# telegraphroad/VCNF

Hardware: AMD Instinct MI355X
Metric: flow transforms/sec (log_prob + sample), D=64 RQ-spline, batch=1M (higher is better)
Workload: dtype f32 results on fp16x3 split operands: every fp32 operand of a conditioner GEMM travels as hi + lo fp16 halves, three f16 matrix instructions per product (four in the 48- and 16-deep layers), fp32 accumulation; measured against fp64 (tests/test_gpu_gemm_error.py): GEMM error 0.6-0.75x the exact-fp32

## Files before the change

### vcnf_amd/csrc/fused_layer_v6.hip

```cpp
#include <hip/hip_runtime.h>
#include <stdint.h>

#include "../../include/vcnf_hip.h"
#include "rqs_math.hpp"
#include "fused_common.hpp"
#include "rqs_lean.hpp"
#include "split_half.hpp"

#ifndef VCNF_ABL
#define VCNF_ABL 0
#endif
#ifndef VCNF_TIME
#define VCNF_TIME 0
#endif
#ifndef VCNF_AHEAD
#define VCNF_AHEAD 1
#endif
#if VCNF_TIME
#define VCNF_T(I) { const long long t_ = clock64(); tacc[I] += t_ - tlast; tlast = t_; }
#define VCNF_TIME_PARAM , float* tstamps
#define VCNF_TIME_ARG , time_buffer()
#else
#define VCNF_T(I)
#define VCNF_TIME_PARAM
#define VCNF_TIME_ARG
#endif

#define VCNF_SYNC() { __builtin_amdgcn_sched_barrier(0); asm volatile("s_waitcnt lgkmcnt(0)\n\ts_barrier" ::: "memory"); __builtin_amdgcn_sched_barrier(0); }

namespace vcnf {

#if VCNF_TIME
constexpr int kTimeSlots = 24;
static float* time_buffer() {
  static float* buf = nullptr;
  if (!buf && hipMalloc(&buf, 2 * kTimeSlots * sizeof(float)) != hipSuccess) buf = nullptr;
  return buf;
}
extern "C" int vcnf_v6_phase_stamps(float* out) {
  if (!time_buffer() || hipDeviceSynchronize() != hipSuccess) return VCNF_ERR_LAUNCH;
  return hipMemcpy(out, time_buffer(), 2 * kTimeSlots * sizeof(float), hipMemcpyDeviceToHost) == hipSuccess ? VCNF_OK : VCNF_ERR_LAUNCH;
}
#endif

template <int DI, int DT, int C, int H, int NBLK, int K, bool INV>
__global__ __launch_bounds__(512, 2) void fused_rqs_layer_v6_kernel(const FusedArgs a VCNF_TIME_PARAM) {
  static_assert(H == 128 && K == 8, "4 row blocks of 32 over 4 waves; 3 K - 1 = 23 logits: two features per 48 rows");
  static_assert((DI == 16 || DI == 32) && DT == DI && (C == 0 || C == 16), "shape family");
  constexpr int kBlock = 512;
  constexpr int kTile = 128;
  constexpr int NCB = 4;
  constexpr int D = DI + DT;
  constexpr int XS = D + 4;
  constexpr int NTX = DI / 16;
  constexpr int NTC = C / 16;
  constexpr int NT0 = NTX + NTC;
  constexpr int NTH = H / 16;
  constexpr int P = 3 * K - 1;
  constexpr int NG = DT / 4;
  constexpr int NR = NG / 2;
  constexpr int TABW = 3 * (K + 1);
  using L = PackLayout6<DI, DT, C, H, NBLK, K>;
  constexpr int GFRAG = 3 * NTH * 2 * 64;
  constexpr int RING = VCNF_AHEAD + 1;

  extern __shared__ __align__(16) float smem[];
  uint4* act = reinterpret_cast<uint4*>(smem);
  uint4* act_hi = act;
  uint4* act_lo = act + NTH * NCB * 64;
  float* xt = smem + 2 * GFRAG * 4;
  uint4* ctxf = reinterpret_cast<uint4*>(xt + kTile * XS);
  float* tab = reinterpret_cast<float*>(ctxf + (C > 0 ? NCB * 2 * 64 : 0));
  float* ldt = tab + ((DI * TABW + 3) & ~3);
  int* tfi = reinterpret_cast<int*>(ldt + kTile);
  int* idi = tfi + DT;
  constexpr int NBV = C > 0 ? 3 : 2;
  constexpr int NBT = 1 + NBLK * NBV;
  constexpr int BPL = NG * 48 + NBT * (H / 2);
  float* biasf = reinterpret_cast<float*>(idi + DI + 4);
  int* tflag = reinterpret_cast<int*>(biasf + 2 * BPL);

  const int tid = threadIdx.x;
  const int lane = tid & 63;
  const int wave = __builtin_amdgcn_readfirstlane(tid >> 6);
  const int rp = wave & 3;
  const int ch = wave >> 2;
  const int c32 = lane & 31;
  const int kg = lane >> 5;
  const RqsConst& c = a.c;
  const bool shared = a.sh_w != nullptr;
  const LeanConst lc = make_lean_const(c);

  if (ch == 1) __builtin_amdgcn_s_setprio(1);
  for (int i = tid; i < NG * 96; i += kBlock) {
    const int g = i / 96, hf = i % 96 / 48;
    biasf[hf * BPL + g * 48 + i % 48] = a.wpack[L::BF + i];
  }
  for (int i = tid; i < NBT * H; i += kBlock) {
    const int v = i / H, blk = (v - 1) / NBV, sel = (v - 1) % NBV, r = i % H;
    const int off = v == 0 ? L::B0 : L::BLK0 + blk * L::BLK + (sel == 0 ? L::BA : sel == 1 ? L::BB : L::BC);
    biasf[(r >> 4 & 1) * BPL + NG * 48 + v * (H / 2) + (r >> 5) * 16 + (r & 15)] = a.wpack[off + r];
  }
  for (int i = tid; i < DT; i += kBlock) tfi[i] = a.tf_idx[i];
  for (int i = tid; i < DI; i += kBlock) idi[i] = a.id_idx[i];
  if (shared) {
    for (int i = tid; i < 3 * DI; i += kBlock) {
      const int f = i % DI;
      SplitLogits p{a.sh_w + f * K, a.sh_h + f * K, a.sh_d + f * (K - 1), K, 1.f, c.edge_logit, c.tails};
      rqs_build_table_part_k<K>(p, c, tab + f * TABW, 1, i / DI);
    }
  }

  const __amdgpu_buffer_rsrc_t wr =
      __builtin_amdgcn_make_buffer_rsrc(const_cast<float*>(a.wpack), 0, a.wpack_bytes, 0x00020000);
  const int voff = lane * 16;
  const float* bplane = biasf + kg * BPL;

  const long long ntiles = (a.B + kTile - 1) / kTile;
  bool bad = false;
  float satm = 0.f;
#if VCNF_TIME
  long long tacc[20], tlast = clock64();
  const long long tstart = tlast, rstart = wall_clock64();
  for (int i = 0; i < 20; ++i) tacc[i] = 0;
#endif
  float4 xpre[kTile * (D / 4) / kBlock], cpre[1];
  static_assert(kTile * (D / 4) % kBlock == 0 && (C == 0 || kTile * (C / 4) == kBlock), "rows per thread");
#define VCNF_PREFETCH_ROWS(TILE)                                                          \
  {                                                                                       \
    const long long pb0 = min((TILE) * kTile, a.B);                                       \
    const long long left = (a.B - pb0) * (D * 4);                                         \
    const __amdgpu_buffer_rsrc_t xr_ = __builtin_amdgcn_make_buffer_rsrc(                 \
        const_cast<float*>(a.x) + pb0 * D, 0, (int)min(left, (long long)(kTile * D * 4)), 0x00020000); \
    _Pragma("unroll") for (int k = 0; k < kTile * (D / 4) / kBlock; ++k)                  \
      xpre[k] = __builtin_bit_cast(float4, __builtin_amdgcn_raw_buffer_load_b128(xr_, (tid + kBlock * k) * 16, 0, 0)); \
    if (C > 0) {                                                                          \
      const long long leftc = (a.B - pb0) * (C * 4);                                      \
      const __amdgpu_buffer_rsrc_t cr_ = __builtin_amdgcn_make_buffer_rsrc(               \
          const_cast<float*>(a.ctx) + pb0 * C, 0, (int)min(leftc, (long long)(kTile * C * 4)), 0x00020000); \
      cpre[0] = __builtin_bit_cast(float4, __builtin_amdgcn_raw_buffer_load_b128(cr_, tid * 16, 0, 0)); \
    }                                                                                     \
  }
  VCNF_PREFETCH_ROWS((long long)blockIdx.x)
  for (long long tile = blockIdx.x; tile < ntiles; tile += gridDim.x) {
    const long long b0 = tile * kTile;
    const int rows = (int)min((long long)kTile, a.B - b0);
    satm = 0.f;
    { VCNF_T(0) VCNF_SYNC(); VCNF_T(15) }
    {
      constexpr int D4 = D / 4;
      if (tid == 0) *tflag = 0;
#pragma unroll
      for (int k = 0; k < kTile * D4 / kBlock; ++k) {
        const int i = tid + kBlock * k;
        const int r = i / D4, o = i - r * D4;
        *reinterpret_cast<float4*>(xt + r * XS + 4 * o) = xpre[k];
      }
      if (C > 0) {
        const int r = tid >> 2, part = tid & 3;
        half4 h4, l4;
        const float cv[4] = {cpre[0].x, cpre[0].y, cpre[0].z, cpre[0].w};
#pragma unroll
        for (int i = 0; i < 4; ++i) satm = fmaxf(satm, cv[i] == cv[i] ? __builtin_fabsf(cv[i]) : __builtin_inff());
        asm volatile("" : "+v"(satm));
#pragma unroll
        for (int i = 0; i < 4; ++i) {
          const float x = __builtin_amdgcn_fmed3f(cv[i], -65504.f, 65504.f);
          const _Float16 hv = (_Float16)x;
          h4[i] = hv;
          l4[i] = (_Float16)((x - (float)hv) * kLoScale);
        }
        const int at = (((r >> 5) * 2) * 64 + (r & 31) + 32 * (part >> 1));
        uint2* dh = reinterpret_cast<uint2*>(ctxf + at) + (part & 1);
        uint2* dl = reinterpret_cast<uint2*>(ctxf + at + 64) + (part & 1);
        *dh = __builtin_bit_cast(uint2, h4);
        *dl = __builtin_bit_cast(uint2, l4);
      }
    }
    { VCNF_T(1) VCNF_SYNC(); VCNF_T(15) }

    {
      constexpr int UNR = DI / 4;
      const int mi = tid >> 2, part = tid & 3;
      float lsum = 0.f;
      float xv[UNR], fv[UNR];
      float* px[UNR];
#pragma unroll
      for (int k = 0; k < UNR; ++k) {
        px[k] = xt + mi * XS + idi[part * UNR + k];
        xv[k] = *px[k];
        fv[k] = xv[k];
      }
      if (shared) {
        float yv[UNR], lad[UNR];
        bool in_[UNR];
#pragma unroll
        for (int k = 0; k < UNR; ++k) {
          in_[k] = (xv[k] >= c.lo_x) && (xv[k] <= c.hi_x);
          bool bad1 = false;
          rqs_point_table_inside<INV, K>(in_[k] ? xv[k] : c.lo_x, tab + (part * UNR + k) * TABW, yv[k], lad[k], bad1);
          bad = bad || (bad1 && in_[k]);
        }
#pragma unroll
        for (int k = 0; k < UNR; ++k) {
          const float o = in_[k] ? yv[k] : xv[k];
          *px[k] = o;
          if (INV) fv[k] = o;
          lsum += in_[k] ? lad[k] : 0.f;
        }
      }
      lsum += __shfl_xor(lsum, 1, 64);
      lsum += __shfl_xor(lsum, 2, 64);
      int tid_ = tid;
      asm volatile("" : "+v"(tid_));
      if (part == 0) ldt[tid_ >> 2] = lsum;
#pragma unroll
      for (int k = 0; k < UNR; ++k) satm = fmaxf(satm, fv[k] == fv[k] ? 0.f : __builtin_inff());
      const int k0 = part * UNR;
      const int t0 = k0 >> 4, kg0 = (k0 >> 3) & 1;
      const int at = (t0 * NCB + (mi >> 5)) * 64 + (mi & 31) + 32 * kg0;
      if (UNR == 8) {
        half8 h8, l8;
        float f8[8];
#pragma unroll
        for (int k = 0; k < 8; ++k) f8[k] = fv[k < UNR ? k : 0];
        split8<false>(f8, h8, l8, satm);
        act_hi[at] = __builtin_bit_cast(uint4, h8);
        act_lo[at] = __builtin_bit_cast(uint4, l8);
      } else {
        half4 h4, l4;
        satm = fmaxf(fmaxf(satm, __builtin_fabsf(fv[0])), __builtin_fabsf(fv[1]));
        satm = fmaxf(fmaxf(satm, __builtin_fabsf(fv[2 < UNR ? 2 : 0])), __builtin_fabsf(fv[3 < UNR ? 3 : 0]));
        asm volatile("" : "+v"(satm));
#pragma unroll
        for (int i = 0; i < 4; ++i) {
          const float x = __builtin_amdgcn_fmed3f(fv[i < UNR ? i : 0], -65504.f, 65504.f);
          const _Float16 hv = (_Float16)x;
          h4[i] = hv;
          l4[i] = (_Float16)((x - (float)hv) * kLoScale);
        }
        reinterpret_cast<uint2*>(act_hi + at)[(k0 >> 2) & 1] = __builtin_bit_cast(uint2, h4);
        reinterpret_cast<uint2*>(act_lo + at)[(k0 >> 2) & 1] = __builtin_bit_cast(uint2, l4);
      }
    }
    { VCNF_T(2) VCNF_SYNC(); VCNF_T(15) }
    if (ch == 1) { VCNF_T(14) VCNF_SYNC(); VCNF_T(16) }

    half8 ahi[NTH], alo[NTH];
    floatx16 abias;
#define VCNF_LOAD_BIAS16(DST, VEC)                                                        \
  _Pragma("unroll") for (int i_ = 0; i_ < 4; ++i_) {                                      \
    const floatx4 b4_ = *reinterpret_cast<const floatx4*>(bplane + NG * 48 + (VEC) * (H / 2) + 16 * rp + 4 * i_); \
    DST[4 * i_ + 0] = b4_[0]; DST[4 * i_ + 1] = b4_[1]; DST[4 * i_ + 2] = b4_[2]; DST[4 * i_ + 3] = b4_[3]; \
  }
#define VCNF_LOAD_HIDDEN(WOFF, BVEC)                                                      \
  {                                                                                       \
    _Pragma("unroll") for (int t = 0; t < NTH; ++t) {                                     \
      ahi[t] = __builtin_bit_cast(half8, wload(wr, voff, 4 * ((WOFF) + ((rp * NTH + t) * 2 + 0) * 256))); \
      alo[t] = __builtin_bit_cast(half8, wload(wr, voff, 4 * ((WOFF) + ((rp * NTH + t) * 2 + 1) * 256))); \
    }                                                                                     \
    VCNF_LOAD_BIAS16(abias, BVEC)                                                         \
  }

    floatx16 h[2];
    {
      half8 w0h[NT0], w0l[NT0];
      floatx16 bias0;
#pragma unroll
      for (int t = 0; t < NT0; ++t) {
        w0h[t] = __builtin_bit_cast(half8, wload(wr, voff, 4 * (L::W0 + ((rp * NT0 + t) * 2 + 0) * 256)));
        w0l[t] = __builtin_bit_cast(half8, wload(wr, voff, 4 * (L::W0 + ((rp * NT0 + t) * 2 + 1) * 256)));
      }
      VCNF_LOAD_BIAS16(bias0, 0)
#pragma unroll
      for (int j = 0; j < 2; ++j) {
        const int cb = 2 * ch + j;
        floatx16 mainv = bias0, corr = {}, corr2 = {};
#pragma unroll
        for (int t = 0; t < NT0; ++t) {
          const half8 bh = __builtin_bit_cast(half8, t < NTX ? act_hi[(t * NCB + cb) * 64 + lane] : ctxf[(cb * 2 + 0) * 64 + lane]);
          const half8 bl = __builtin_bit_cast(half8, t < NTX ? act_lo[(t * NCB + cb) * 64 + lane] : ctxf[(cb * 2 + 1) * 64 + lane]);
          mainv = mfma32h(w0h[t], bh, mainv);
          corr = mfma32h(w0h[t], bl, corr);
          corr = mfma32h(w0l[t], bh, corr);
          corr2 = mfma32h(w0l[t], bl, corr2);
        }
#pragma unroll
        for (int r = 0; r < 16; ++r) h[j][r] = fmaf(fmaf(corr2[r], kLoUnscale, corr[r]), kLoUnscale, mainv[r]);
      }
    }
    { VCNF_T(3) VCNF_SYNC(); VCNF_T(15) }
#define VCNF_PUBLISH(SRC, RELU)                                                           \
  _Pragma("unroll") for (int j = 0; j < 2; ++j) {                                         \
    _Pragma("unroll") for (int hh = 0; hh < 2; ++hh) {                                    \
      float v8_[8];                                                                       \
      _Pragma("unroll") for (int i = 0; i < 8; ++i) v8_[i] = SRC[j][8 * hh + i];          \
      half8 h8_, l8_;                                                                     \
      split8<RELU>(v8_, h8_, l8_, satm);                                                  \
      const int at = ((2 * rp + hh) * NCB + 2 * ch + j) * 64 + lane;                      \
      act_hi[at] = __builtin_bit_cast(uint4, h8_);                                        \
      act_lo[at] = __builtin_bit_cast(uint4, l8_);                                        \
    }                                                                                     \
  }
    VCNF_LOAD_HIDDEN(L::BLK0 + L::WA, 1)
    VCNF_PUBLISH(h, true)
    { VCNF_T(4) VCNF_SYNC(); VCNF_T(15) }

#define VCNF_READ_B(T)                                                                    \
  {                                                                                       \
    rh[(T) % RING] = __builtin_bit_cast(half8, act_hi[((((T) & 7)) * NCB + 2 * ch + ((T) >> 3)) * 64 + lane]); \
    rl[(T) % RING] = __builtin_bit_cast(half8, act_lo[((((T) & 7)) * NCB + 2 * ch + ((T) >> 3)) * 64 + lane]); \
  }
#define VCNF_HIDDEN_COMPUTE(OUT)                                                          \
  {                                                                                       \
    half8 rh[RING], rl[RING];                 \
    floatx16 corr;                                                                        \
    _Pragma("unroll") for (int st_ = 0; st_ < VCNF_AHEAD; ++st_) {                        \
      VCNF_READ_B(st_)                                                                    \
    }                                                                                     \
    _Pragma("unroll") for (int st_ = 0; st_ < 2 * NTH; ++st_) {                           \
      const int j = st_ >> 3, tk_ = st_ & 7;                                              \
      if (st_ + VCNF_AHEAD < 2 * NTH) {                                                   \
        VCNF_READ_B(st_ + VCNF_AHEAD)                                                     \
      }                                                                                   \
      if (tk_ == 0) {                                                                       \
        OUT[j] = abias;                                                                   \
        corr = floatx16{};                                                                \
      }                                                                                   \
      OUT[j] = mfma32h(ahi[tk_], rh[st_ % RING], OUT[j]);                                      \
      corr = mfma32h(ahi[tk_], rl[st_ % RING], corr);                                          \
      corr = mfma32h(alo[tk_], rh[st_ % RING], corr);                                          \
      if (tk_ == NTH - 1) {                                                                 \
        _Pragma("unroll") for (int r = 0; r < 16; ++r) OUT[j][r] = fmaf(corr[r], kLoUnscale, OUT[j][r]); \
      }                                                                                   \
    }                                                                                     \
    __builtin_amdgcn_sched_group_barrier(0x100, 2 * VCNF_AHEAD, 0);                       \
    _Pragma("unroll") for (int st_ = 0; st_ + VCNF_AHEAD < 2 * NTH; ++st_) {              \
      __builtin_amdgcn_sched_group_barrier(0x100, 2, 0);                                  \
      __builtin_amdgcn_sched_group_barrier(0x008, 3, 0);                                  \
    }                                                                                     \
    __builtin_amdgcn_sched_group_barrier(0x008, 3 * VCNF_AHEAD, 0);                       \
  }

#pragma unroll
    for (int blk = 0; blk < (VCNF_ABL == 5 ? 0 : NBLK); ++blk) {
      const int base = L::BLK0 + blk * L::BLK;
      floatx16 t[2];
      VCNF_HIDDEN_COMPUTE(t)
      { VCNF_T(5) VCNF_SYNC(); VCNF_T(15) }
      VCNF_LOAD_HIDDEN(base + L::WB, 2 + blk * NBV)
      half8 wch, wcl;
      floatx16 gate[2], gbias;
      if (C > 0) {
        wch = __builtin_bit_cast(half8, wload(wr, voff, 4 * (base + L::WC + (rp * 2 + 0) * 256)));
        wcl = __builtin_bit_cast(half8, wload(wr, voff, 4 * (base + L::WC + (rp * 2 + 1) * 256)));
        VCNF_LOAD_BIAS16(gbias, 3 + blk * NBV)
      }
      VCNF_PUBLISH(t, true)
      { VCNF_T(6) VCNF_SYNC(); VCNF_T(15) }
      VCNF_HIDDEN_COMPUTE(t)
      if (C > 0 && VCNF_ABL != 6) {
#pragma unroll
        for (int j = 0; j < 2; ++j) {
          const half8 bh = __builtin_bit_cast(half8, ctxf[((2 * ch + j) * 2 + 0) * 64 + lane]);
          const half8 bl = __builtin_bit_cast(half8, ctxf[((2 * ch + j) * 2 + 1) * 64 + lane]);
          floatx16 corr = {}, corr2 = {};
          gate[j] = mfma32h(wch, bh, gbias);
          corr = mfma32h(wch, bl, corr);
          corr = mfma32h(wcl, bh, corr);
          corr2 = mfma32h(wcl, bl, corr2);
#pragma unroll
          for (int r = 0; r < 16; ++r) gate[j][r] = fmaf(fmaf(corr2[r], kLoUnscale, corr[r]), kLoUnscale, gate[j][r]);
        }
      }
      { VCNF_T(5) VCNF_SYNC(); VCNF_T(15) }
      if (blk + 1 < NBLK) {
        VCNF_LOAD_HIDDEN(base + L::BLK + L::WA, 1 + (blk + 1) * NBV)
      }
      if (C > 0 && VCNF_ABL != 6) {
#pragma unroll
        for (int j = 0; j < 2; ++j) {
#pragma unroll
          for (int r = 0; r < 16; ++r) {
            const float sg = hw_rcp(1.f + hw_exp2(-gate[j][r]));
            h[j][r] = fmaf(t[j][r], sg, h[j][r]);
          }
        }
      } else {
#pragma unroll
        for (int j = 0; j < 2; ++j) h[j] += t[j];
      }
      if (blk + 1 < NBLK) {
        VCNF_PUBLISH(h, true)
      } else {
        VCNF_PUBLISH(h, false)
      }
      { VCNF_T(7) VCNF_SYNC(); VCNF_T(15) }
    }
    if (ch == 0) { VCNF_T(14) VCNF_SYNC(); VCNF_T(17) }
#undef VCNF_HIDDEN_COMPUTE
#undef VCNF_READ_B
#undef VCNF_LOAD_HIDDEN
#undef VCNF_PUBLISH

    half8 fhi[NTH], flo[NTH];
#pragma unroll
    for (int t = 0; t < NTH; ++t) {
      fhi[t] = __builtin_bit_cast(half8, act_hi[(t * NCB + rp) * 64 + lane]);
      flo[t] = __builtin_bit_cast(half8, act_lo[(t * NCB + rp) * 64 + lane]);
    }
    float ld_acc = 0.f;
    uint4* win = act + ch * GFRAG;
    const int gtid = tid & 255;
    constexpr int NSTG = GFRAG / 256;
    static_assert(GFRAG % 256 == 0, "whole fragments per thread");
#define VCNF_STAGE_DMA(G)                                                                 \
  _Pragma("unroll") for (int k = 0; k < NSTG; ++k)                                        \
    dma16_to_lds(wr, win + (gtid & ~63) + k * 256, gtid * 16, 4 * (L::WF + (G) * (4 * GFRAG) + k * 1024));
    floatx16 pa[3];
#define VCNF_LOAD_BIASF(G)                                                                \
  _Pragma("unroll") for (int b = 0; b < 3; ++b) {                                         \
    _Pragma("unroll") for (int i_ = 0; i_ < 4; ++i_) {                                    \
      const floatx4 b4_ = *reinterpret_cast<const floatx4*>(bplane + (G) * 48 + 16 * b + 4 * i_); \
      pa[b][4 * i_ + 0] = b4_[0]; pa[b][4 * i_ + 1] = b4_[1]; pa[b][4 * i_ + 2] = b4_[2]; pa[b][4 * i_ + 3] = b4_[3]; \
    }                                                                                     \
  }
    VCNF_LOAD_BIASF(ch)
    { VCNF_T(8) VCNF_SYNC(); VCNF_T(15) }
    VCNF_STAGE_DMA(ch)
    wait_vector_memory();
    { VCNF_T(9) VCNF_SYNC(); VCNF_T(15) }
    if (ch == 1) { VCNF_T(14) VCNF_SYNC(); VCNF_T(18) }
    for (int rnd = 0; rnd < (VCNF_ABL == 3 ? 0 : NR); ++rnd) {
      const int g = 2 * rnd + ch;
      float* px[2];
      float xin[2];
#pragma unroll
      for (int f2 = 0; f2 < 2; ++f2) {
        px[f2] = xt + (rp * 32 + c32) * XS + tfi[4 * g + 2 * kg + f2];
        xin[f2] = *px[f2];
      }
      {
        half8 wh[RING], wl[RING];
        floatx16 corr;
#define VCNF_READ_W(T)                                                                    \
  {                                                                                       \
    wh[(T) % RING] = __builtin_bit_cast(half8, win[((T) * 2 + 0) * 64 + lane]);           \
    wl[(T) % RING] = __builtin_bit_cast(half8, win[((T) * 2 + 1) * 64 + lane]);           \
  }
#pragma unroll
        for (int u = 0; u < VCNF_AHEAD; ++u) {
          VCNF_READ_W(u)
        }
#pragma unroll
        for (int u = 0; u < 3 * NTH; ++u) {
          const int b = u >> 3, t = u & 7;
          if (u + VCNF_AHEAD < 3 * NTH) {
            VCNF_READ_W(u + VCNF_AHEAD)
          }
          if (t == 0) corr = floatx16{};
          pa[b] = mfma32h(wh[u % RING], fhi[t], pa[b]);
          corr = mfma32h(wh[u % RING], flo[t], corr);
          corr = mfma32h(wl[u % RING], fhi[t], corr);
          if (t == NTH - 1) {
#pragma unroll
            for (int r = 0; r < 16; ++r) pa[b][r] = fmaf(corr[r], kLoUnscale, pa[b][r]);
          }
        }
        __builtin_amdgcn_sched_group_barrier(0x100, 2 * VCNF_AHEAD, 0);
#pragma unroll
        for (int u = 0; u + VCNF_AHEAD < 3 * NTH; ++u) {
          __builtin_amdgcn_sched_group_barrier(0x100, 2, 0);
          __builtin_amdgcn_sched_group_barrier(0x008, 3, 0);
        }
        __builtin_amdgcn_sched_group_barrier(0x008, 3 * VCNF_AHEAD, 0);
#undef VCNF_READ_W
      }
      { VCNF_T(10) VCNF_SYNC(); VCNF_T(15) }
      {
        const bool more = rnd + 1 < NR;
        if (!more) {
          VCNF_PREFETCH_ROWS(tile + gridDim.x)
        }
        if (more && VCNF_ABL != 2) {
          VCNF_STAGE_DMA(g + 2)
        }
        float yv[2], lad[2];
#pragma unroll
        for (int f2 = 0; f2 < 2; ++f2) {
          float lg[P];
#pragma unroll
          for (int tl = 0; tl < P; ++tl) lg[tl] = pa[(24 * f2 + tl) >> 4][(24 * f2 + tl) & 15];
          rqs_lean_eval<8, INV>(xin[f2], lg, lc, yv[f2], lad[f2], bad);
        }
        *px[0] = yv[0];
        *px[1] = yv[1];
        ld_acc += lad[0] + lad[1];
        if (more) {
          VCNF_LOAD_BIASF(g + 2)
        }
      }
      if (rnd + 1 < NR && VCNF_ABL != 2) wait_vector_memory();
      { VCNF_T(11) VCNF_SYNC(); VCNF_T(15) }
    }
    if (ch == 0) { VCNF_T(14) VCNF_SYNC(); VCNF_T(19) }
#undef VCNF_PREFETCH_ROWS
#undef VCNF_STAGE_DMA
#undef VCNF_LOAD_BIASF

    ld_acc += __shfl_xor(ld_acc, 32, 64);
    if (ch == 1 && kg == 0) ldt[rp * 32 + c32] += ld_acc;
    if (satm > 65504.f) *tflag = 1;
    { VCNF_T(12) VCNF_SYNC(); VCNF_T(15) }
    const bool over = *tflag != 0;
    if (tid == 0 && over && a.sat) atomicAdd(a.sat, 1);
    if (a.redo && tid < kTile / kFusedFlagRows && b0 + tid * kFusedFlagRows < a.B)
      a.redo[tile * (kTile / kFusedFlagRows) + tid] = over ? 1 : 0;
    if (over && a.redo) continue;
    if (ch == 0 && kg == 0) {
      const int mrow = rp * 32 + c32;
      if (mrow < rows) {
        const float o = a.ld_sign * (ld_acc + ldt[mrow]);
        a.logdet[b0 + mrow] = a.ld_mode ? a.logdet[b0 + mrow] + o : o;
      }
    }
    {
      constexpr int D4 = D / 4;
      float4* dst = reinterpret_cast<float4*>(a.y) + b0 * D4;
      for (int i = tid; i < rows * D4; i += kBlock) {
        const int r = i / D4, o = i - r * D4;
        dst[i] = *reinterpret_cast<const float4*>(xt + r * XS + 4 * o);
      }
    }
  }
#if VCNF_TIME
  VCNF_T(13)
  if (blockIdx.x == 0 && (tid & 255) == 0 && tstamps) {
    float* ts = tstamps + (tid >> 8) * kTimeSlots;
    for (int i = 0; i < 20; ++i) ts[i] = (float)tacc[i];
    ts[20] = (float)(clock64() - tstart);
    ts[21] = (float)(wall_clock64() - rstart);
    ts[22] = (float)((ntiles - blockIdx.x + gridDim.x - 1) / gridDim.x);
  }
#endif
  if (INV && a.bad && bad) atomicAdd(a.bad, 1);
}

template <int DI, int DT, int C, int H, int NBLK, int K>
static int launch_v6(const FusedArgs& a, int inverse, hipStream_t st) {
  constexpr int D = DI + DT;
  constexpr int TILE = 128;
  constexpr size_t WIN = (size_t)2 * 3 * (H / 16) * 2 * 64 * 16;
  constexpr int NBT = 1 + NBLK * (C > 0 ? 3 : 2);
  const size_t lds = ((size_t)TILE * (D + 4) + ((DI * 3 * (K + 1) + 3) & ~3) + TILE + D + 8 + (DT / 4) * 96 + NBT * H) * 4 +
                     (C > 0 ? 4 * 2 * 64 * 16 : 0) + WIN + 64;
  static bool attr_set[2] = {false, false};
  if (!attr_set[inverse ? 1 : 0]) {
    hipError_t e;
    if (inverse)
      e = hipFuncSetAttribute(reinterpret_cast<const void*>(&fused_rqs_layer_v6_kernel<DI, DT, C, H, NBLK, K, true>),
                              hipFuncAttributeMaxDynamicSharedMemorySize, (int)lds);
    else
      e = hipFuncSetAttribute(reinterpret_cast<const void*>(&fused_rqs_layer_v6_kernel<DI, DT, C, H, NBLK, K, false>),
                              hipFuncAttributeMaxDynamicSharedMemorySize, (int)lds);
    if (e != hipSuccess) return VCNF_ERR_LAUNCH;
    attr_set[inverse ? 1 : 0] = true;
  }
  const long long ntiles = (a.B + TILE - 1) / TILE;
  dim3 grid((unsigned)(ntiles < 256 ? ntiles : 256));
  if (inverse)
    hipLaunchKernelGGL((fused_rqs_layer_v6_kernel<DI, DT, C, H, NBLK, K, true>), grid, dim3(512), lds, st, a VCNF_TIME_ARG);
  else
    hipLaunchKernelGGL((fused_rqs_layer_v6_kernel<DI, DT, C, H, NBLK, K, false>), grid, dim3(512), lds, st, a VCNF_TIME_ARG);
  return hipGetLastError() == hipSuccess ? VCNF_OK : VCNF_ERR_LAUNCH;
}

template <int NBLK>
static int launch_v6_family(const FusedArgs& a, int d_id, int ctx_dim, int inverse, hipStream_t st) {
#ifdef VCNF_DEV_ONLY
  return launch_v6<32, 32, 16, 128, NBLK, 8>(a, inverse, st);
#else
  if (d_id == 32) {
    return ctx_dim == 16 ? launch_v6<32, 32, 16, 128, NBLK, 8>(a, inverse, st)
                         : launch_v6<32, 32, 0, 128, NBLK, 8>(a, inverse, st);
  }
  return ctx_dim == 16 ? launch_v6<16, 16, 16, 128, NBLK, 8>(a, inverse, st)
                       : launch_v6<16, 16, 0, 128, NBLK, 8>(a, inverse, st);
#endif
}

#ifndef VCNF_V6_NBLK
#define VCNF_V6_NBLK 2
#endif
#if VCNF_V6_NBLK == 1
int launch_fused_v6_b1(const FusedArgs& a, int d_id, int ctx_dim, int inverse, hipStream_t st) {
  return launch_v6_family<1>(a, d_id, ctx_dim, inverse, st);
}
#elif VCNF_V6_NBLK == 2
int launch_fused_v6_b2(const FusedArgs& a, int d_id, int ctx_dim, int inverse, hipStream_t st) {
  return launch_v6_family<2>(a, d_id, ctx_dim, inverse, st);
}
#else
int launch_fused_v6_b3(const FusedArgs& a, int d_id, int ctx_dim, int inverse, hipStream_t st) {
  return launch_v6_family<3>(a, d_id, ctx_dim, inverse, st);
}
#endif

}
```

Before: 75.88 million.

## Buffer-store tile epilogue, prefetch old logdet into LDS, pin prefetched rows

Measured after the change: 76.73 million, median of 6. 1.1% higher.

```diff
diff --git a/vcnf_amd/csrc/fused_layer_v6.hip b/vcnf_amd/csrc/fused_layer_v6.hip
--- a/vcnf_amd/csrc/fused_layer_v6.hip
+++ b/vcnf_amd/csrc/fused_layer_v6.hip
@@ -78,7 +78,8 @@
   constexpr int NBT = 1 + NBLK * NBV;
   constexpr int BPL = NG * 48 + NBT * (H / 2);
   float* biasf = reinterpret_cast<float*>(idi + DI + 4);
-  int* tflag = reinterpret_cast<int*>(biasf + 2 * BPL);
+  float* ldold = biasf + 2 * BPL;
+  int* tflag = reinterpret_cast<int*>(ldold + kTile);
 
   const int tid = threadIdx.x;
   const int lane = tid & 63;
@@ -141,7 +142,21 @@
       cpre[0] = __builtin_bit_cast(float4, __builtin_amdgcn_raw_buffer_load_b128(cr_, tid * 16, 0, 0)); \
     }                                                                                     \
   }
+#define VCNF_ROWS_ARRIVED()                                                               \
+  {                                                                                       \
+    _Pragma("unroll") for (int k = 0; k < kTile * (D / 4) / kBlock; ++k) {                \
+      floatx4 v_ = __builtin_bit_cast(floatx4, xpre[k]);                                  \
+      asm volatile("" : "+v"(v_));                                                        \
+      xpre[k] = __builtin_bit_cast(float4, v_);                                           \
+    }                                                                                     \
+    if (C > 0) {                                                                          \
+      floatx4 v_ = __builtin_bit_cast(floatx4, cpre[0]);                                  \
+      asm volatile("" : "+v"(v_));                                                        \
+      cpre[0] = __builtin_bit_cast(float4, v_);                                           \
+    }                                                                                     \
+  }
   VCNF_PREFETCH_ROWS((long long)blockIdx.x)
+  VCNF_ROWS_ARRIVED()
   for (long long tile = blockIdx.x; tile < ntiles; tile += gridDim.x) {
     const long long b0 = tile * kTile;
     const int rows = (int)min((long long)kTile, a.B - b0);
@@ -428,6 +443,11 @@
     VCNF_LOAD_BIASF(ch)
     { VCNF_T(8) VCNF_SYNC(); VCNF_T(15) }
     VCNF_STAGE_DMA(ch)
+    if (ch == 0 && rp < 2 && a.ld_mode) {
+      const __amdgpu_buffer_rsrc_t or_ = __builtin_amdgcn_make_buffer_rsrc(a.logdet + b0, 0, rows * 4, 0x00020000);
+      __builtin_amdgcn_raw_ptr_buffer_load_lds(or_, (__attribute__((address_space(3))) void*)(ldold + rp * 64), 4,
+                                               lane * 4, rp * 256, 0, 0);
+    }
     wait_vector_memory();
     { VCNF_T(9) VCNF_SYNC(); VCNF_T(15) }
     if (ch == 1) { VCNF_T(14) VCNF_SYNC(); VCNF_T(18) }
@@ -512,25 +532,39 @@
     if (ch == 1 && kg == 0) ldt[rp * 32 + c32] += ld_acc;
     if (satm > 65504.f) *tflag = 1;
     { VCNF_T(12) VCNF_SYNC(); VCNF_T(15) }
+    VCNF_ROWS_ARRIVED()
+#undef VCNF_ROWS_ARRIVED
+    int tid_ = tid;
+    asm volatile("" : "+v"(tid_));
     const bool over = *tflag != 0;
     if (tid == 0 && over && a.sat) atomicAdd(a.sat, 1);
-    if (a.redo && tid < kTile / kFusedFlagRows && b0 + tid * kFusedFlagRows < a.B)
-      a.redo[tile * (kTile / kFusedFlagRows) + tid] = over ? 1 : 0;
-    if (over && a.redo) continue;
-    if (ch == 0 && kg == 0) {
-      const int mrow = rp * 32 + c32;
-      if (mrow < rows) {
-        const float o = a.ld_sign * (ld_acc + ldt[mrow]);
-        a.logdet[b0 + mrow] = a.ld_mode ? a.logdet[b0 + mrow] + o : o;
-      }
+    if (a.redo) {
+      if (tid_ < kTile / kFusedFlagRows) {
+        const __amdgpu_buffer_rsrc_t rr = __builtin_amdgcn_make_buffer_rsrc(
+            a.redo + tile * (kTile / kFusedFlagRows), 0, 4 * ((rows + kFusedFlagRows - 1) / kFusedFlagRows), 0x00020000);
+        __builtin_amdgcn_raw_buffer_store_b32(over ? 1 : 0, rr, tid_ * 4, 0, 0);
+      }
+      if (over) continue;
+    }
+    if (ch == 0 && (tid_ & 32) == 0) {
+      const int mrow = (tid_ >> 6) * 32 + (tid_ & 31);
+      const __amdgpu_buffer_rsrc_t lr = __builtin_amdgcn_make_buffer_rsrc(a.logdet + b0, 0, rows * 4, 0x00020000);
+      const float o = a.ld_sign * (ld_acc + ldt[mrow]);
+      __builtin_amdgcn_raw_buffer_store_b32(__builtin_bit_cast(unsigned, a.ld_mode ? ldold[mrow] + o : o), lr, mrow * 4, 0, 0);
     }
     {
       constexpr int D4 = D / 4;
-      float4* dst = reinterpret_cast<float4*>(a.y) + b0 * D4;
-      for (int i = tid; i < rows * D4; i += kBlock) {
+      const __amdgpu_buffer_rsrc_t yr = __builtin_amdgcn_make_buffer_rsrc(a.y + b0 * D, 0, rows * (D * 4), 0x00020000);
+      floatx4 yv[kTile * D4 / kBlock];
+#pragma unroll
+      for (int k = 0; k < kTile * D4 / kBlock; ++k) {
+        const int i = tid_ + kBlock * k;
         const int r = i / D4, o = i - r * D4;
-        dst[i] = *reinterpret_cast<const float4*>(xt + r * XS + 4 * o);
-      }
+        yv[k] = *reinterpret_cast<const floatx4*>(xt + r * XS + 4 * o);
+      }
+#pragma unroll
+      for (int k = 0; k < kTile * D4 / kBlock; ++k)
+        __builtin_amdgcn_raw_buffer_store_b128(__builtin_bit_cast(__attribute__((ext_vector_type(4))) unsigned, yv[k]), yr, (tid_ + kBlock * k) * 16, 0, 0);
     }
   }
 #if VCNF_TIME
@@ -552,7 +586,7 @@
   constexpr int TILE = 128;
   constexpr size_t WIN = (size_t)2 * 3 * (H / 16) * 2 * 64 * 16;
   constexpr int NBT = 1 + NBLK * (C > 0 ? 3 : 2);
-  const size_t lds = ((size_t)TILE * (D + 4) + ((DI * 3 * (K + 1) + 3) & ~3) + TILE + D + 8 + (DT / 4) * 96 + NBT * H) * 4 +
+  const size_t lds = ((size_t)TILE * (D + 4) + ((DI * 3 * (K + 1) + 3) & ~3) + 2 * TILE + D + 8 + (DT / 4) * 96 + NBT * H) * 4 +
                      (C > 0 ? 4 * 2 * 64 * 16 : 0) + WIN + 64;
   static bool attr_set[2] = {false, false};
   if (!attr_set[inverse ? 1 : 0]) {
```
